# boguszjelinski/taxidispatcher

Hardware: AMD Instinct MI355X
Metric: NxN assignments/sec (higher is better)
Workload: dtype int32; 1 GPU; g1 N=16384: device cost write (4N^2 B) + exact assignment, total checked == optimum; n=16384, parallelism=single GPU

## Files before the change

taxidispatcher_amd/csrc/td_assign.hip:

```cpp
#include <dlfcn.h>
#include <limits.h>
#include <stdlib.h>

#include <type_traits>

#include "td_common.h"

using namespace td;

namespace {

template <typename CT>
struct Tr;
template <>
struct Tr<uint8_t> {
    using PT = int32_t;
    static constexpr int E = 16;
    static constexpr uint32_t SENT = 0xFFu;
    static constexpr int64_t LIMIT = 254;
    static constexpr int32_t BIG = 1 << 28;
    static constexpr int32_t KMAX = INT32_MAX;
};
template <>
struct Tr<uint16_t> {
// ... 830 lines not shown
        bk = s_k[wb];
        bp = s_p[wb];
        x = s_x[wb];
        for (int k = 0; k < 4; k++)
            if (k != wb && s_k[k] < x) x = s_k[k];
        if (bp != INT_MAX) {
            const int t1 = bp / E;
            int ch = t1 + rot;
            if (ch >= nchunks) ch -= nchunks;
            const int j1 = ch * E + (bp - t1 * E);
            const PT inc = (x == Tr<CT>::KMAX) ? (PT)0 : (PT)((x >> 1) - (bk >> 1));
            const bool owned = (bk & 1) != 0;
            if (j1 < n && (!(owned && inc == 0) || tie_evict)) {
                const PT newp = (P[j1] >> 1) + inc;
                atomicMax(&bid[j1], ((unsigned long long)newp << ROW_BITS) | (unsigned long long)(row + 1));
            }
        }
    }
    __syncthreads();
    }
}

template <typename PT>
__global__ __launch_bounds__(256) void k_assign(int n, int nrows, int row0, unsigned long long *__restrict__ bid,
                                                PT *__restrict__ pk, int *__restrict__ owner, int *__restrict__ r2c,
                                                int *__restrict__ ctl, int round, long long plimit = 0 )
{
    if (ctl[CTL_FLAG]) return;
    if (round > 0 && round < 60 && ctl[CTL_PROG + round - 1] == 0) return;
    const int j = blockIdx.x * blockDim.x + threadIdx.x;
    int cnt = 0;
    if (j < n) {
        const unsigned long long k = bid[j];
        if (k) {
            const int row = (int)(k & ((1ull << ROW_BITS) - 1)) - 1;
            const PT newp = (PT)(k >> ROW_BITS);
            if (plimit && (long long)(k >> ROW_BITS) >= plimit) atomicOr(&ctl[CTL_FLAG], 8);
            const int old = owner[j];
            const PT oldp = pk[j] >> 1;
            if (old >= row0 && old < row0 + nrows) r2c[old - row0] = -1;
            owner[j] = row;
            if (row >= row0 && row < row0 + nrows) r2c[row - row0] = j;
            pk[j] = (PT)(newp << 1) | (PT)1;
            bid[j] = 0ull;
            cnt = (old < 0 || newp > oldp) ? 1 : 0;
        }
    }
    const unsigned long long m = __ballot(cnt);
    if ((threadIdx.x & 63) == 0 && m) {
        if (round < 60) atomicAdd(&ctl[CTL_PROG + round], (int)__popcll(m));
    }
}

__device__ __forceinline__ int build_free_list(int n, const int *__restrict__ r2c, int *__restrict__ list, int want = -1)
{
    __shared__ int s_fl_w[16];
    __shared__ int s_fl_tot;
    const int T = blockDim.x, tid = threadIdx.x, lane = tid & 63, w = tid >> 6, nw = T >> 6;
    const int per = (n + T - 1) / T;
    const int lo = tid * per, hi = min(n, lo + per);
    int cnt = 0;
    const bool vec = (per & 3) == 0 && (reinterpret_cast<uintptr_t>(r2c) & 15) == 0;
    if (vec) {
        int r = lo;
#pragma unroll 4
        for (; r + 4 <= hi; r += 4) {
            const int4 x = *reinterpret_cast<const int4 *>(r2c + r);
            cnt += (x.x == want) + (x.y == want) + (x.z == want) + (x.w == want);
        }
        for (; r < hi; r++) cnt += (r2c[r] == want) ? 1 : 0;
    } else
        for (int r = lo; r < hi; r++) cnt += (r2c[r] == want) ? 1 : 0;
    int incl = cnt;
#pragma unroll
    for (int o = 1; o < 64; o <<= 1) {
        const int v = __shfl_up(incl, o);
        if (lane >= o) incl += v;
    }
    if (lane == 63) s_fl_w[w] = incl;
    __syncthreads();
    int base = 0;
    for (int k = 0; k < w; k++) base += s_fl_w[k];
    if (tid == T - 1) s_fl_tot = base + incl;
    int pos = base + incl - cnt;
    if (cnt) {
        if (vec) {
            int r = lo;
            for (; r + 4 <= hi; r += 4) {
                const int4 x = *reinterpret_cast<const int4 *>(r2c + r);
                if (x.x == want) list[pos++] = r;
                if (x.y == want) list[pos++] = r + 1;
                if (x.z == want) list[pos++] = r + 2;
                if (x.w == want) list[pos++] = r + 3;
            }
            for (; r < hi; r++)
                if (r2c[r] == want) list[pos++] = r;
        } else
            for (int r = lo; r < hi; r++)
                if (r2c[r] == want) list[pos++] = r;
    }
    __syncthreads();
    const int tot = s_fl_tot;
    __syncthreads();
    return tot;
}

__global__ __launch_bounds__(1024) void k_freelist(int n, const int *__restrict__ r2c, int *__restrict__ list,
                                                   int *__restrict__ ctl)
{
    if (ctl[CTL_FLAG]) return;
    const int cnt = build_free_list(n, r2c, list);
    if (threadIdx.x == 0) ctl[CTL_NFREE] = cnt;
}

#include "td_blocks.h"
#include "td_core_warm.h"

__device__ __forceinline__ void place_const_tail(int n, int *__restrict__ r2c, int *__restrict__ owner,
                                                 int *__restrict__ lista, int *__restrict__ listb,
                                                 int *__restrict__ ctl)
{
    if (ctl[CTL_NCONST] == 0) return;
    const int nr = build_free_list(n, r2c, lista, -2);
    if (nr == 0) return;
    const int nc = build_free_list(n, owner, listb, -1);
    if (nc != nr) {
        if (threadIdx.x == 0) atomicOr(&ctl[CTL_ERR], 8);
        return;
    }
    for (int k = threadIdx.x; k < nr; k += blockDim.x) {
        const int r = lista[k], j = listb[k];
        r2c[r] = j;
        owner[j] = r;
    }
}

__global__ __launch_bounds__(1024) void k_place_const(int n, int *__restrict__ r2c, int *__restrict__ owner,
                                                      int *__restrict__ lista, int *__restrict__ listb,
                                                      int *__restrict__ ctl, const int *__restrict__ gate_left = nullptr)
{
    if (ctl[CTL_FLAG]) return;
    if (gate_left && *gate_left != 0) return;
    place_const_tail(n, r2c, owner, lista, listb, ctl);
}

__device__ __forceinline__ void shape_decide(int n, int *__restrict__ ctl)
{
    int *sh = ctl + CTL_SHAPE;
    __threadfence();
    const int ncol = atomicAdd(&sh[0], 0);
    const int nrow = atomicAdd(&ctl[CTL_NCONST], 0);
    sh[1] = nrow;
    const int margin = n / 256 > 32 ? n / 256 : 32;
    if (ncol >= 16 && ncol - nrow >= margin) {
        sh[3] = 1;
        atomicOr(&ctl[CTL_FLAG], 4);
    }
}

__device__ __forceinline__ void shape_probe(int n, const int32_t *__restrict__ cost, int *__restrict__ ctl, int tickets)
{
    int *sh = ctl + CTL_SHAPE;
    const int t = blockIdx.x * blockDim.x + threadIdx.x;
    int cc = 0;
    long long rng = 0;
    if (t < n) {
        const int v0 = cost[t];
        int mn = v0, mx = v0;
#pragma unroll
        for (int k = 1; k < 16; k++) {
            const int v = cost[(int64_t)(((int64_t)k * n) >> 4) * n + t];
            mn = min(mn, v);
            mx = max(mx, v);
        }
        cc = (mn == mx) ? 1 : 0;
        rng = (long long)mx - (long long)mn;
    }
#pragma unroll
    for (int o = 32; o > 0; o >>= 1) {
        cc += __shfl_xor(cc, o);
        const long long orng = __shfl_xor(rng, o);
        rng = orng > rng ? orng : rng;
    }
    if ((threadIdx.x & 63) == 0) {
        if (cc) atomicAdd(&sh[0], cc);
        if (rng > 254) atomicMax(reinterpret_cast<unsigned long long *>(&sh[4]), (unsigned long long)rng);
    }
    __shared__ int s_last;
    __syncthreads();
    if (threadIdx.x == 0) {
        __threadfence();
        s_last = (atomicAdd(&sh[2], 1) == tickets - 1);
    }
    __syncthreads();
    if (s_last && threadIdx.x == 0) shape_decide(n, ctl);
// ... 1490 lines not shown
        for (int k = lane; k < rc->plen; k += 64) ok = ok && (touch[rc->path[k]] == r);
        for (int k = lane; k < rc->nS; k += 64) ok = ok && (pthm[rc->S_col[k]] >= r);
        if (__ballot(!ok)) continue;
        for (int k = lane; k < rc->nS; k += 64) {
            const int col = rc->S_col[k];
            const unsigned long long rv = atomicExch(&raise[col], 0ull);
            if (rv) {
                if (plimit && (long long)(pk[col] >> 1) + (long long)rv >= plimit) atomicOr(&ctl[CTL_FLAG], 8);
                pk[col] = pk[col] + (PT)((PT)rv << 1);
            }
        }
        if (lane == 0) pk[rc->endcol] = pk[rc->endcol] | (PT)1;
    }
    __syncthreads();
    const int nleft = build_free_list(n, r2c, list);
    if (tid == 0) s_nfree = nleft;
    __syncthreads();
    if (tid == 0) {
        ctl[CTL_NFREE] = s_nfree;
        if (!first && s_acc == 0) ctl[CTL_PSTOP] = 1;
        ctl[CTL_PACC] += s_acc;
    }
}

__device__ __forceinline__ void fin_record(const int *ctl, const unsigned long long *out, const int *left, unsigned int *ticket, int *rec)
{
    __shared__ int s_last;
    __syncthreads();
    if (threadIdx.x == 0) {
        __threadfence();
        s_last = atomicAdd(ticket, 1u) == gridDim.x - 1;
    }
    __syncthreads();
    if (!s_last) return;
    __threadfence();
    for (int k = threadIdx.x; k < CTL_ALL; k += blockDim.x) rec[k] = __hip_atomic_load(ctl + k, __ATOMIC_RELAXED, __HIP_MEMORY_SCOPE_AGENT);
    if (threadIdx.x == 0) {
        long long *rt = reinterpret_cast<long long *>(reinterpret_cast<char *>(rec) + FIN_OFF);
        rt[0] = (long long)__hip_atomic_load(out, __ATOMIC_RELAXED, __HIP_MEMORY_SCOPE_AGENT);
        rt[1] = (long long)__hip_atomic_load(out + 1, __ATOMIC_RELAXED, __HIP_MEMORY_SCOPE_AGENT);
        rec[REC_LEFT / sizeof(int)] = __hip_atomic_load(left, __ATOMIC_RELAXED, __HIP_MEMORY_SCOPE_AGENT);
        *ticket = 0u;
    }
}

template <bool GEN = false>
__global__ __launch_bounds__(256) void k_final(int n, int nrows, int row0, const int32_t *__restrict__ cost,
                                               const int *__restrict__ r2c, const int *__restrict__ owner,
                                               unsigned long long *__restrict__ out, int *__restrict__ ctl, int cost_is_transposed = 0,
                                               const CellSrc src = CellSrc(), const int *__restrict__ gate_left = nullptr,
                                               int *__restrict__ r2c_out = nullptr, unsigned int *__restrict__ ticket = nullptr,
                                               int *__restrict__ rec = nullptr)
{
    const bool go = !ctl[CTL_FLAG] && !(gate_left && *gate_left != 0);
    if (go) {
    long long s = 0;
    int bad = 0;
    for (int i = blockIdx.x * blockDim.x + threadIdx.x; i < nrows; i += gridDim.x * blockDim.x) {
        const int j = r2c[i];
        if (r2c_out) r2c_out[i] = j;
        if (j < 0 || j >= n || owner[j] != row0 + i)
            bad = 1;
        else
            s += GEN ? (long long)(cost_is_transposed ? src.cell(j, i) : src.cell(i, j))
                     : (long long)(cost_is_transposed ? cost[(int64_t)j * n + i] : cost[(int64_t)i * n + j]);
    }
#pragma unroll
    for (int o = 32; o > 0; o >>= 1) {
        s += __shfl_xor(s, o);
        bad |= __shfl_xor(bad, o);
    }
    if ((threadIdx.x & 63) == 0) {
        atomicAdd(&out[0], (unsigned long long)s);
        if (bad) atomicOr(&ctl[CTL_ERR], 4);
    }
    }
    if (rec) fin_record(ctl, out, gate_left, ticket, rec);
}

__global__ void k_pack_totals(const long long *__restrict__ tot2, const int *__restrict__ ctl, long long *__restrict__ out3)
{
    if (threadIdx.x == 0) {
        out3[0] = tot2[0];
        out3[1] = tot2[1];
        out3[2] = (long long)(ctl[CTL_ERR] != 0) + (long long)(ctl[CTL_FLAG] != 0);
    }
}

__global__ void k_r2c_from_owner(int n, int nrows, int row0, const int *__restrict__ owner, int *__restrict__ r2c)
{
    const int j = blockIdx.x * blockDim.x + threadIdx.x;
    if (j < n) {
        const int o = owner[j];
        if (o >= row0 && o < row0 + nrows) r2c[o - row0] = j;
    }
}

__global__ void k_const_mask(int row0, int nrows, const int *__restrict__ rconst, int *__restrict__ mask_full)
{
    const int i = blockIdx.x * blockDim.x + threadIdx.x;
    if (i < nrows && rconst[i]) mask_full[row0 + i] = 1;
}

__global__ __launch_bounds__(1024) void k_mark_const(int n, const int *__restrict__ mask, int *__restrict__ r2c_full, int *__restrict__ ctl)
{
    __shared__ int s_cnt;
    if (threadIdx.x == 0) s_cnt = 0;
    __syncthreads();
    int cnt = 0;
    for (int i = threadIdx.x; i < n; i += blockDim.x)
        if (mask[i]) {
            r2c_full[i] = -2;
            cnt++;
        }
#pragma unroll
    for (int o = 32; o > 0; o >>= 1) cnt += __shfl_xor(cnt, o);
    if ((threadIdx.x & 63) == 0 && cnt) atomicAdd(&s_cnt, cnt);
    __syncthreads();
    if (threadIdx.x == 0) ctl[CTL_NCONST] = s_cnt;
}

template <typename PT>
__global__ void k_price_io(int n, PT *pk, long long *plain, int set)
{
    const int j = blockIdx.x * blockDim.x + threadIdx.x;
    if (j < n) {
        if (set)
            pk[j] = (PT)((PT)plain[j] << 1) | (PT)1;
        else
            plain[j] = (long long)(pk[j] >> 1);
    }
}

__global__ void k_fill_i32(int *p, int count, int v)
{
    const int i = blockIdx.x * blockDim.x + threadIdx.x;
    if (i < count) p[i] = v;
}

template <typename CT>
__global__ __launch_bounds__(256) void k_dual(int n, int nrows, int row0, int nchunks, const CT *__restrict__ cc,
                                              const typename Tr<CT>::PT *__restrict__ pk,
                                              const int32_t *__restrict__ rowmin, unsigned long long *__restrict__ out,
                                              const int *__restrict__ gate_left = nullptr, const int *__restrict__ ctl = nullptr)
{
    using PT = typename Tr<CT>::PT;
    constexpr int E = Tr<CT>::E;
    if (gate_left && (*gate_left != 0 || ctl[CTL_FLAG] != 0)) return;
    const int lane = threadIdx.x & 63, w = threadIdx.x >> 6, nw = blockDim.x >> 6;
    const size_t pitch = (size_t)nchunks * E;
    long long acc = 0;
    for (int row = blockIdx.x * nw + w; row < nrows; row += gridDim.x * nw) {
        const CT *rp = cc + (size_t)row * pitch;
        PT m = Tr<CT>::KMAX;
        for (int ch = lane; ch < nchunks; ch += 64) {
            const uint4 cv = *reinterpret_cast<const uint4 *>(rp + (size_t)ch * E);
            uint32_t c[E];
            unpack<CT>(cv, c);
#pragma unroll
            for (int e = 0; e < E; e++) {
                const PT v = (PT)c[e] + (pk[(size_t)ch * E + e] >> 1);
                m = v < m ? v : m;
            }
        }
#pragma unroll
        for (int o = 32; o > 0; o >>= 1) {
            PT om = shfl_xor_t(m, o);
            m = om < m ? om : m;
        }
        if (lane == 0) acc += (long long)m + (long long)rowmin[row];
    }
    if (blockIdx.x == 0 && row0 == 0) {
        long long ps = 0;
        for (int j = threadIdx.x; j < n; j += blockDim.x) ps += (long long)(pk[j] >> 1);
#pragma unroll
        for (int o = 32; o > 0; o >>= 1) ps += __shfl_xor(ps, o);
        if (lane == 0) acc -= ps;
    }
    if (lane == 0 && acc != 0) atomicAdd(&out[1], (unsigned long long)acc);
}

}

struct td_shard {
    int n = 0, row0 = 0, nrows = 0;
    int bpc = 0;
    int64_t range = 0;
    int64_t fit_bound = -1;
    int nchunks = 0, npad = 0;
    const int32_t *d_cost = nullptr;
    Buf stage, cc, price, owner, r2c, r2c_full, bid, pred, list, rowmin, rconst, misc, psrec, tbuf, xbuf, fbuf;
    bool defer_const = false;
    int nconst = -1;
    const int32_t *probe = nullptr;
    bool placed = false;
    int64_t range_seen = -1;
    bool want_bid0 = false;
    bool bid0_done = false;
    Buf cmask;
    bool have_cmask = false;
    bool fused_t = false;
// ... 254 lines not shown
    HopCtl *hc = (HopCtl *)sv.hop.p;
    int *frl = (int *)sv.list.p, *fcl = (int *)sv.pred.p;
    const int *ctl = (const int *)sv.misc.p;
    if (gate && nb != 1) return fail(TD_EINTERNAL, "a gated two-hop pass takes one block");
    const int nseg = raw && window_zero ? (ncols_blk / 4 + 1023) / 1024 : 1;
    k_hop_lists<<<nb, 1024, 0, c.stream>>>(rpb, ncols_blk, col_lo, (const int *)sv.r2c.p, (const int *)sv.owner.p, frl, fcl, hc, ctl,
                                           gate ? g_hop_max_rows : 0, nseg > 1 ? (int *)sv.hoptab.p : nullptr);
    if (raw) {
        if (!sv.d_cost || sv.n % 4) return fail(TD_EINVAL, "two-hop pass on the int32 matrix: no matrix, or n %% 4 != 0");
        if (nseg > 1)
            k_hop_table<CT, true, true><<<nb * HOP_FMAX * nseg, 256, 0, c.stream>>>(
                sv.n, sv.nrows, sv.row0, sv.n / 4, rpb, ncols_blk, col_lo, g_hop_max_rows, 1, (const CT *)sv.d_cost, (const PT *)sv.price.p,
                (const int *)sv.owner.p, frl, fcl, hc, (int *)sv.hoptab.p, ctl, (const int32_t *)sv.rowmin.p, nseg);
        else
        k_hop_table<CT, true><<<nb * HOP_FMAX, 256, 0, c.stream>>>(sv.n, sv.nrows, sv.row0, sv.n / 4, rpb, ncols_blk, col_lo, g_hop_max_rows,
                                                                   window_zero ? 1 : 0, (const CT *)sv.d_cost, (const PT *)sv.price.p,
                                                                   (const int *)sv.owner.p, frl, fcl, hc, (int *)sv.hoptab.p, ctl,
                                                                   (const int32_t *)sv.rowmin.p);
    } else {
    k_hop_table<CT><<<nb * HOP_FMAX, 256, 0, c.stream>>>(sv.n, sv.nrows, sv.row0, sv.nchunks, rpb, ncols_blk, col_lo, g_hop_max_rows,
                                                         window_zero ? 1 : 0, (const CT *)sv.cc.p, (const PT *)sv.price.p,
                                                         (const int *)sv.owner.p, frl, fcl, hc, (int *)sv.hoptab.p, ctl);
    }
    const size_t match_lds = sizeof(uint32_t) * ((size_t)HOP_FMAX * HOP_FMAX + (size_t)((rpb + 31) / 32));
    if (match_lds > 150 * 1024) return fail(TD_EINVAL, "two-hop pass: a block of that many rows does not fit the LDS");
    TD_HIP(hipFuncSetAttribute((const void *)k_hop_match<PT>, hipFuncAttributeMaxDynamicSharedMemorySize, (int)match_lds));
    k_hop_match<PT><<<nb, HOP_MATCH_T, match_lds, c.stream>>>(
        sv.nrows, sv.row0, rpb, ncols_blk, col_lo, g_hop_max_rows, (PT *)sv.price.p, (int *)sv.owner.p, (int *)sv.r2c.p, ob, frl, fcl, hc,
        (const int *)sv.hoptab.p, (int *)sv.misc.p);
    TD_HIP(hipGetLastError());
    return TD_OK;
}

int sv_phase_a(Solver &sv, int hop_passes)
{
    Ctx &c = ctx();
    const int n = sv.n, nrows = sv.nrows;
    const int rpb = n / sv.zs_V, nb = nrows / rpb;
    const int col_lo = (sv.row0 / rpb) * rpb, col_hi = col_lo + nb * rpb;
    int rc;
    if ((rc = ensure(sv.ob, (size_t)sv.npad + 64))) return rc;
    if (!sv.ob_clear) TD_HIP(hipMemsetAsync(sv.ob.p, 0, (size_t)sv.npad, c.stream));
    sv.ob_clear = false;
    ProfScope ps(TD_K_BID);
    int *ctl = (int *)sv.misc.p;
    const int ga = (col_hi - col_lo + 255) / 256;
    unsigned long long *bid = (unsigned long long *)sv.bid.p;
    auto assign = [&]() {
        k_zs_assign<<<ga, 256, 0, c.stream>>>(col_lo, col_hi, nrows, sv.row0, bid, (int32_t *)sv.price.p, (int *)sv.owner.p, (int *)sv.r2c.p,
                                              (uint8_t *)sv.ob.p, ctl);
    };
    assign();
    for (int r = 1; r <= g_zs_rounds; r++) {
        k_zs_bid<<<std::min(nrows, c.n_cu * 16), 256, 0, c.stream>>>(nrows, sv.row0, sv.nchunks, rpb, (const uint8_t *)sv.cc.p,
                                                                     (const uint8_t *)sv.ob.p, (const int *)sv.r2c.p, bid, ctl, r, g_tie_evict);
        assign();
    }
    TD_HIP(hipGetLastError());
    for (int p = 0; p < hop_passes; p++)
        if ((rc = sv_hop_t<uint8_t>(sv, rpb, rpb, col_lo, nb, true, (uint8_t *)sv.ob.p))) return rc;
    if (getenv("TD_DEBUG") && hop_passes > 0) {
        HopCtl h;
        TD_HIP(hipMemcpyAsync(&h, sv.hop.p, sizeof(h), hipMemcpyDeviceToHost, c.stream));
        TD_HIP(hipStreamSynchronize(c.stream));
        fprintf(stderr, "[td] phase A: %d blocks of %d rows, %d local rounds; free rows / columns per block before the last two-hop pass:", nb, rpb, g_zs_rounds);
        for (int b = 0; b < nb; b++) fprintf(stderr, " %d/%d", h.nfr[b], h.nfc[b]);
        fprintf(stderr, " | matched %d, left %d\n", h.matched, h.left);
    }
    sv.zs_done = false;
    sv.bid0_done = false;
    sv.state_ready = true;
    return TD_OK;
}

template <typename CT>
int sv_begin_t(Solver &sv)
{
    Ctx &c = ctx();
    using PT = typename Tr<CT>::PT;
    const PT padkey = (PT)(Tr<CT>::BIG << 1) | (PT)1;
    k_init_state<PT><<<(std::max(sv.npad, (int)CTL_WORDS) + 255) / 256, 256, 0, c.stream>>>(
        sv.n, sv.npad, sv.nrows, (PT *)sv.price.p, padkey, (int *)sv.owner.p, (int *)sv.r2c.p,
        (unsigned long long *)sv.bid.p, (int *)sv.misc.p, sv.defer_const ? (const int *)sv.rconst.p : nullptr, sv.probe, 0, nullptr,
        g_one_trip ? (unsigned long long *)((char *)sv.misc.p + FIN_OFF) : nullptr);
    if (!g_one_trip) TD_HIP(hipMemsetAsync((char *)sv.misc.p + FIN_OFF, 0, 16, c.stream));
    TD_HIP(hipGetLastError());
    sv.began = true;
    return TD_OK;
}

template <typename CT>
int sv_bid_t(Solver &sv, int r, unsigned long long *keys)
{
    Ctx &c = ctx();
    using PT = typename Tr<CT>::PT;
    const int n = sv.n, nrows = sv.nrows;
    if (nrows == 0) return TD_OK;
    const size_t lds_prices = (size_t)sv.npad * sizeof(PT);
    const bool can_lds = lds_prices <= 128 * 1024 && n >= 2048 && nrows >= 1024;
    const int tie_evict = (r >= 1) ? g_tie_evict : 0;
    ProfScope ps(TD_K_BID);
    int *tied = (r == 0) ? (int *)sv.misc.p + CTL_TIED : nullptr;
    const bool sparse = sv.state_ready;
    if (can_lds && r < g_lds_rounds && !sparse) {
        if (lds_prices > 48 * 1024)
            (void)hipFuncSetAttribute((const void *)k_bid<CT, true>, hipFuncAttributeMaxDynamicSharedMemorySize, (int)lds_prices);
        const int grid = std::min((nrows + 15) / 16, c.n_cu * g_lds_grid);
// ... 1783 lines not shown
```

taxidispatcher_amd/csrc/td_blocks.h:

```cpp


struct HopCtl {
    int nfr[HOP_BMAX], nfc[HOP_BMAX];
    int left;
    int matched;
    int pad[2];
};

__device__ __forceinline__ uint32_t zs_zero_bytes(uint32_t w)
{
    return ~(((w & 0x7F7F7F7Fu) + 0x7F7F7F7Fu) | w | 0x7F7F7F7Fu);
}

__global__ __launch_bounds__(256) void k_zs_bid(int nrows, int row0, int nchunks, int rpb, const uint8_t *__restrict__ cc,
                                                const uint8_t *__restrict__ ob, const int *__restrict__ r2c,
                                                unsigned long long *__restrict__ bid, const int *__restrict__ ctl, int round,
                                                int tie_evict)
{
    __shared__ int s_best[4];
    if (ctl[CTL_FLAG]) return;
    const int tid = threadIdx.x, lane = tid & 63, w = tid >> 6;
    const int cpb = rpb >> 4;
    const size_t pitch = (size_t)nchunks * 16;
    for (int lrow = blockIdx.x; lrow < nrows; lrow += gridDim.x) {
        if (r2c[lrow] != -1) continue;
        const int row = row0 + lrow;
        const int c0 = (row / rpb) * cpb;
        const uint32_t hsh = ((uint32_t)row + 1u) * 0x9E3779B1u + (uint32_t)round * 0x85EBCA6Bu;
        const int rot = (int)(((uint64_t)(hsh ^ (hsh >> 15)) * (uint64_t)cpb) >> 32);
        const uint8_t *rp = cc + (size_t)lrow * pitch;
        int best = INT_MAX;
        for (int t = tid; t < cpb; t += 256) {
            int ch = t + rot;
            if (ch >= cpb) ch -= cpb;
            ch += c0;
            const uint4 cv = *reinterpret_cast<const uint4 *>(rp + (size_t)ch * 16);
            const uint4 ov = *reinterpret_cast<const uint4 *>(ob + (size_t)ch * 16);
            const uint32_t cw[4] = {cv.x, cv.y, cv.z, cv.w}, ow[4] = {ov.x, ov.y, ov.z, ov.w};
#pragma unroll
            for (int k = 0; k < 4; k++) {
                const uint32_t z = zs_zero_bytes(cw[k]);
                if (!z) continue;
                const uint32_t zf = z & zs_zero_bytes(ow[k]);
                const uint32_t pick = zf ? zf : z;
                const int cand = (zf ? 0 : (1 << 24)) | (t * 16 + k * 4 + (__builtin_ctz(pick) >> 3));
                best = min(best, cand);
            }
        }
#pragma unroll
        for (int o = 32; o > 0; o >>= 1) best = min(best, __shfl_xor(best, o));
        if (lane == 0) s_best[w] = best;
        __syncthreads();
        if (tid == 0) {
            best = min(min(s_best[0], s_best[1]), min(s_best[2], s_best[3]));
            if (best != INT_MAX) {
                const bool owned = (best >> 24) != 0;
                const int pos = best & 0xFFFFFF;
                int ch = (pos >> 4) + rot;
                if (ch >= cpb) ch -= cpb;
                const int j = (c0 + ch) * 16 + (pos & 15);
                if (!owned || tie_evict) atomicMax(&bid[j], (unsigned long long)(row + 1));
            }
        }
        __syncthreads();
    }
}

__global__ __launch_bounds__(256) void k_zs_assign(int col_lo, int col_hi, int nrows, int row0, unsigned long long *__restrict__ bid,
                                                   int32_t *__restrict__ pk, int *__restrict__ owner, int *__restrict__ r2c,
                                                   uint8_t *__restrict__ ob, const int *__restrict__ ctl)
{
    if (ctl[CTL_FLAG]) return;
    const int j = col_lo + blockIdx.x * blockDim.x + threadIdx.x;
    if (j >= col_hi) return;
    const unsigned long long k = bid[j];
    if (!k) return;
    const int row = (int)(k & ((1ull << ROW_BITS) - 1)) - 1;
    const int old = owner[j];
    if (old >= row0 && old < row0 + nrows) r2c[old - row0] = -1;
    owner[j] = row;
    if (row >= row0 && row < row0 + nrows) r2c[row - row0] = j;
    pk[j] = 1;
    ob[j] = 1;
    bid[j] = 0ull;
}

constexpr int HOP_NONE = INT_MAX;
__global__ __launch_bounds__(1024) void k_hop_lists(int rpb, int ncols_blk, int col_lo, const int *__restrict__ r2c,
                                                    const int *__restrict__ owner, int *__restrict__ frl, int *__restrict__ fcl,
                                                    HopCtl *__restrict__ hc, const int *__restrict__ ctl, int gate_max = 0,
                                                    int *__restrict__ tab_preset = nullptr)
{
    if (ctl[CTL_FLAG]) return;
    const int lb = blockIdx.x;
    if (gate_max > 0) {
        __shared__ int s_go;
        if (threadIdx.x == 0) {
            const int left = hc->left;
            s_go = left > 0 && left <= gate_max;
        }
        __syncthreads();
        if (!s_go) {
            if (threadIdx.x == 0) hc->nfr[lb] = 0, hc->nfc[lb] = 0;
            return;
        }
    }
    const int nfr = build_free_list(rpb, r2c + (size_t)lb * rpb, frl + (size_t)lb * rpb, -1);
    const int nfc = build_free_list(ncols_blk, owner + col_lo + (size_t)lb * ncols_blk, fcl + (size_t)lb * ncols_blk, -1);
    if (threadIdx.x == 0) {
        hc->nfr[lb] = nfr;
        hc->nfc[lb] = nfc;
        if (lb == 0) hc->left = 0, hc->matched = 0;
    }
    if (tab_preset) {
        int4 *t4 = reinterpret_cast<int4 *>(tab_preset + (size_t)lb * HOP_FMAX * HOP_FMAX);
        for (int k = threadIdx.x; k < min(nfr, HOP_FMAX) * (HOP_FMAX / 4); k += 1024) t4[k] = make_int4(HOP_NONE, HOP_NONE, HOP_NONE, HOP_NONE);
    }
}

template <typename CT, bool RAW = false, bool SPLIT = false>
__global__ __launch_bounds__(256) void k_hop_table(int n, int nrows, int row0, int nchunks, int rpb, int ncols_blk, int col_lo,
                                                   int max_rows, int window_zero, const CT *__restrict__ cc,
                                                   const typename Tr<CT>::PT *__restrict__ pk, const int *__restrict__ owner,
                                                   const int *__restrict__ frl, const int *__restrict__ fcl,
                                                   const HopCtl *__restrict__ hc, int *__restrict__ tab,
                                                   const int *__restrict__ ctl, const int32_t *__restrict__ rowmin = nullptr,
                                                   int nseg = 1)
{
    using PT = typename Tr<CT>::PT;
    constexpr int E = RAW ? 4 : Tr<CT>::E;
    __shared__ int s_tab[HOP_FMAX];
    constexpr int CHT = RAW ? 4 : 1;
    __shared__ int s_cand[256 * E * CHT];
    __shared__ int s_hr[256 * E * CHT], s_hj[256 * E * CHT];
    __shared__ int s_fc[HOP_FMAX];
    __shared__ int s_ncand, s_nhit;
    __shared__ long long s_v[4];
    constexpr int HU = 4;
    if (ctl[CTL_FLAG]) return;
    const int seg = SPLIT ? (int)blockIdx.x % nseg : 0, ba = SPLIT ? (int)blockIdx.x / nseg : (int)blockIdx.x;
    const int lb = ba / HOP_FMAX, a = ba % HOP_FMAX;
    const int nfr = hc->nfr[lb];
    if (nfr > max_rows || a >= min(nfr, HOP_FMAX)) return;
    const int tid = threadIdx.x, lane = tid & 63, w = tid >> 6;
    const int lrow = lb * rpb + frl[(size_t)lb * rpb + a];
    const size_t pitch = (size_t)nchunks * E;
    const unsigned char *rp = reinterpret_cast<const unsigned char *>(cc) + (size_t)lrow * pitch * (RAW ? 4 : sizeof(CT));
    const int32_t mn = RAW ? rowmin[lrow] : 0;
    auto cells = [&](const uint4 &raw, uint32_t *c) {
        if constexpr (RAW) {
            c[0] = (uint32_t)((int32_t)raw.x - mn), c[1] = (uint32_t)((int32_t)raw.y - mn);
            c[2] = (uint32_t)((int32_t)raw.z - mn), c[3] = (uint32_t)((int32_t)raw.w - mn);
        } else
            unpack<CT>(raw, c);
    };
    auto ecell = [&](int rl, int col) -> long long {
        if constexpr (RAW) return (long long)(uint32_t)(reinterpret_cast<const int32_t *>(cc)[(size_t)rl * pitch + col] - rowmin[rl]);
        else return (long long)(uint32_t)cc[(size_t)rl * pitch + col];
    };
    const int nfc = min(hc->nfc[lb], HOP_FMAX);
    const int cb = col_lo + lb * ncols_blk;
    if (tid < nfc) s_fc[tid] = fcl[(size_t)lb * ncols_blk + tid];
    int *tab_row = tab + ((size_t)lb * HOP_FMAX + a) * HOP_FMAX;
    if (!SPLIT && tid < HOP_FMAX) s_tab[tid] = INT_MAX;
    if (tid == 0) s_ncand = 0, s_nhit = 0;
    const int ch_lo = window_zero ? (col_lo + lb * ncols_blk) / E : 0;
    const int ch_n = window_zero ? (ncols_blk + E - 1) / E : nchunks;
    long long v = 0;
    if (!window_zero) {
        long long mv = LLONG_MAX;
        for (int t = tid; t < ch_n; t += 256) {
            uint32_t c[E];
            cells(*reinterpret_cast<const uint4 *>(rp + (size_t)(ch_lo + t) * 16), c);
            PT pv[E];
            const int j0 = (ch_lo + t) * E;
            if constexpr (sizeof(PT) == 4) {
                const int4 *pp = reinterpret_cast<const int4 *>(pk + j0);
#pragma unroll
                for (int q = 0; q < E / 4; q++) {
                    const int4 x = pp[q];
                    pv[4 * q + 0] = x.x, pv[4 * q + 1] = x.y, pv[4 * q + 2] = x.z, pv[4 * q + 3] = x.w;
                }
            } else {
#pragma unroll
                for (int e = 0; e < E; e++) pv[e] = pk[j0 + e];
            }
#pragma unroll
            for (int e = 0; e < E; e++)
                if (j0 + e < n) mv = min(mv, (long long)c[e] + (long long)(pv[e] >> 1));
        }
#pragma unroll
        for (int o = 32; o > 0; o >>= 1) {
            const long long ov = __shfl_xor(mv, o);
            mv = ov < mv ? ov : mv;
        }
        if (lane == 0) s_v[w] = mv;
        __syncthreads();
        v = min(min(s_v[0], s_v[1]), min(s_v[2], s_v[3]));
    }
    __syncthreads();
    for (int t0 = SPLIT ? seg * 256 * CHT : 0; t0 < (SPLIT ? min(ch_n, (seg + 1) * 256 * CHT) : ch_n); t0 += 256 * CHT) {
        uint4 raws[CHT];
#pragma unroll
        for (int u = 0; u < CHT; u++) {
            const int t = t0 + u * 256 + tid;
            if (t < ch_n) raws[u] = *reinterpret_cast<const uint4 *>(rp + (size_t)(ch_lo + t) * 16);
        }
#pragma unroll
        for (int u = 0; u < CHT; u++) {
        const int t = t0 + u * 256 + tid;
        if (t < ch_n) {
            const uint4 raw = raws[u];
            bool any = true;
            if constexpr (!RAW && sizeof(CT) == 1 && std::is_same<CT, uint8_t>::value)
                if (window_zero) any = (zs_zero_bytes(raw.x) | zs_zero_bytes(raw.y) | zs_zero_bytes(raw.z) | zs_zero_bytes(raw.w)) != 0;
// ... 22 lines not shown
        }
        }
        __syncthreads();
        const int nc = s_ncand;
        for (int k = tid; k < nc; k += 256) {
            const int j = s_cand[k], r = owner[j];
            if (r < row0 || r >= row0 + nrows) continue;
            if ((r - row0) / rpb != lb) continue;
            const int h = atomicAdd(&s_nhit, 1);
            s_hr[h] = r - row0, s_hj[h] = j;
        }
        __syncthreads();
        const int np = s_nhit * nfc;
        int *dst = SPLIT ? tab_row : s_tab;
        for (int p0 = 0; p0 < np; p0 += 256 * HU) {
            long long du[HU], dx[HU];
            int rg[HU], bb[HU];
            bool live[HU];
#pragma unroll
            for (int q = 0; q < HU; q++) {
                const int p = min(p0 + q * 256 + tid, np - 1);
                const int h = p / nfc, b = p - h * nfc;
                const int rl = s_hr[h], j = s_hj[h], jb = cb + s_fc[b];
                rg[q] = rl + row0, bb[q] = b;
                live[q] = SPLIT || s_tab[b] > rg[q];
                du[q] = dx[q] = 0;
                if (live[q]) {
                    du[q] = ecell(rl, j) + (long long)(pk[j] >> 1);
                    dx[q] = ecell(rl, jb) + (long long)(pk[jb] >> 1);
                }
            }
#pragma unroll
            for (int q = 0; q < HU; q++)
                if (live[q] && p0 + q * 256 + tid < np && du[q] == dx[q]) atomicMin(&dst[bb[q]], rg[q]);
        }
        __syncthreads();
        if (tid == 0) s_ncand = 0, s_nhit = 0;
        __syncthreads();
    }
    if (!SPLIT && tid < HOP_FMAX) tab_row[tid] = s_tab[tid] == INT_MAX ? -1 : s_tab[tid];
}

constexpr int HOP_MATCH_T = 256;
template <typename PT>
__global__ __launch_bounds__(HOP_MATCH_T) void k_hop_match(int nrows, int row0, int rpb, int ncols_blk, int col_lo, int max_rows,
                                                           PT *__restrict__ pk, int *__restrict__ owner, int *__restrict__ r2c,
                                                           uint8_t *__restrict__ ob, const int *__restrict__ frl,
                                                           const int *__restrict__ fcl, HopCtl *__restrict__ hc,
                                                           const int *__restrict__ tab, int *__restrict__ ctl)
{
    extern __shared__ uint32_t s_hop_dyn[];
    __shared__ int s_st[HOP_FMAX];
    __shared__ int s_win[HOP_FMAX][2];
    if (ctl[CTL_FLAG]) return;
    const int lb = blockIdx.x;
    const int nfr = hc->nfr[lb];
    const int tid = threadIdx.x;
    if (nfr == 0) return;
    if (nfr > max_rows) {
        if (tid == 0) atomicAdd(&hc->left, nfr);
        return;
    }
    const int na = min(nfr, HOP_FMAX), nc = min(hc->nfc[lb], HOP_FMAX);
    int *s_tab = reinterpret_cast<int *>(s_hop_dyn);
    uint32_t *s_usedr = s_hop_dyn + HOP_FMAX * HOP_FMAX;
    const int *fr = frl + (size_t)lb * rpb, *fc = fcl + (size_t)lb * ncols_blk;
    const int blk_row0 = row0 + lb * rpb;
    const int my_i = tid < na ? blk_row0 + fr[tid] : 0;
    {
        const int4 *src = reinterpret_cast<const int4 *>(tab + (size_t)lb * HOP_FMAX * HOP_FMAX);
        int4 *dst = reinterpret_cast<int4 *>(s_tab);
        auto norm = [&](int r, int col) { return (r == HOP_NONE || col >= nc) ? -1 : r; };
        for (int k = tid; k < na * (HOP_FMAX / 4); k += HOP_MATCH_T) {
            const int4 x = src[k];
            const int col = (k * 4) & (HOP_FMAX - 1);
            dst[k] = make_int4(norm(x.x, col), norm(x.y, col + 1), norm(x.z, col + 2), norm(x.w, col + 3));
        }
        for (int k = tid; k < (rpb + 31) / 32; k += HOP_MATCH_T) s_usedr[k] = 0u;
        if (tid < na) {
            const uint32_t hsh = ((uint32_t)my_i + 1u) * 0x9E3779B1u;
            s_st[tid] = nc ? (int)(((uint64_t)(hsh ^ (hsh >> 15)) * (uint64_t)nc) >> 32) : 0;
        }
    }
    __syncthreads();
    if (tid < 64) {
        const int lane = tid;
        auto entry = [&](int a, int col) -> int {
            const int r = s_tab[min(a, HOP_FMAX - 1) * HOP_FMAX + col];
            return a < na ? r : -1;
        };
        auto used = [&](int r) -> bool {
            const int rb = max(r - blk_row0, 0);
            const uint32_t word = s_usedr[rb >> 5];
            return r < 0 || ((word >> (rb & 31)) & 1u);
        };
        unsigned long long usedc0 = 0ull, usedc1 = 0ull;
        int done = 0, r_prev = -1;
        int ra0 = entry(0, lane), ra1 = entry(0, lane + 64);
        int rb0 = entry(1, lane), rb1 = entry(1, lane + 64);
        bool ua0 = used(ra0), ua1 = used(ra1);
        int st = s_st[0];
        for (int a = 0; a < na; a++) {
            const int rc0 = entry(a + 2, lane), rc1 = entry(a + 2, lane + 64);
            const bool ub0 = used(rb0), ub1 = used(rb1);
            const int st_nx = s_st[min(a + 1, HOP_FMAX - 1)];
            const unsigned long long m0 = __ballot(!ua0 && ra0 != r_prev) & ~usedc0;
            const unsigned long long m1 = __ballot(!ua1 && ra1 != r_prev) & ~usedc1;
            int rw = -1, cw = 0;
            if (m0 | m1) {
                const unsigned long long h0 = st < 64 ? m0 & (~0ull << st) : 0ull;
                const unsigned long long h1 = st < 64 ? m1 : m1 & (~0ull << (st - 64));
                if (h0 | h1) cw = h0 ? __builtin_ctzll(h0) : 64 + __builtin_ctzll(h1);
                else cw = m0 ? __builtin_ctzll(m0) : 64 + __builtin_ctzll(m1);
                rw = __builtin_amdgcn_readlane(cw < 64 ? ra0 : ra1, cw & 63);
                if (cw < 64) usedc0 |= 1ull << cw;
                else usedc1 |= 1ull << (cw - 64);
                r_prev = rw;
                done++;
            }
            if (lane == 0) {
                s_win[a][0] = rw, s_win[a][1] = cw;
                if (rw >= 0) {
                    const int rb = rw - blk_row0;
                    atomicOr(&s_usedr[rb >> 5], 1u << (rb & 31));
                }
            }
            __builtin_amdgcn_fence(__ATOMIC_ACQ_REL, "wavefront");
            ra0 = rb0, ra1 = rb1, ua0 = ub0, ua1 = ub1;
            rb0 = rc0, rb1 = rc1;
// ... 22 lines not shown
```

Baseline: 29.38 million assignments/s.

## Hoist control-flag loads and batch independent loads across small assignment kernels

Several small kernels (zero-slack bid, bid apply, hop free-list, hop table, hop match, final check, place_const) now issue their control-flag reads together with the first data loads, so the latencies overlap instead of running in series. k_zs_bid is remapped to one wavefront per row with no shared-memory barriers and two chunks in flight per lane. The grid grows to one block per four rows. The free-list builder fuses the row and column counting passes and their prefix scans into a single pass. This adds speculative loads, clamped indices and a larger launch grid, and it leans on empty asm statements to force load ordering.

```diff
diff --git a/taxidispatcher_amd/csrc/td_assign.hip b/taxidispatcher_amd/csrc/td_assign.hip
--- a/taxidispatcher_amd/csrc/td_assign.hip
+++ b/taxidispatcher_amd/csrc/td_assign.hip
@@ -906,16 +906,18 @@
     }
 }
 
-__device__ __forceinline__ int build_free_list(int n, const int *__restrict__ r2c, int *__restrict__ list, int want = -1)
-{
-    __shared__ int s_fl_w[16];
-    __shared__ int s_fl_tot;
-    const int T = blockDim.x, tid = threadIdx.x, lane = tid & 63, w = tid >> 6, nw = T >> 6;
+__device__ __forceinline__ bool free_list_vec(int n, const int *r2c)
+{
+    return (((n + (int)blockDim.x - 1) / (int)blockDim.x) & 3) == 0 && (reinterpret_cast<uintptr_t>(r2c) & 15) == 0;
+}
+
+__device__ __forceinline__ int free_list_count(int n, const int *__restrict__ r2c, int want)
+{
+    const int T = blockDim.x, tid = threadIdx.x;
     const int per = (n + T - 1) / T;
     const int lo = tid * per, hi = min(n, lo + per);
     int cnt = 0;
-    const bool vec = (per & 3) == 0 && (reinterpret_cast<uintptr_t>(r2c) & 15) == 0;
-    if (vec) {
+    if (free_list_vec(n, r2c)) {
         int r = lo;
 #pragma unroll 4
         for (; r + 4 <= hi; r += 4) {
@@ -925,6 +927,71 @@
         for (; r < hi; r++) cnt += (r2c[r] == want) ? 1 : 0;
     } else
         for (int r = lo; r < hi; r++) cnt += (r2c[r] == want) ? 1 : 0;
+    return cnt;
+}
+
+__device__ __forceinline__ void free_list_count2(int n, const int *__restrict__ a, int wanta, const int *__restrict__ b, int wantb,
+                                                 int &cnta, int &cntb)
+{
+    const int T = blockDim.x, tid = threadIdx.x;
+    const int per = (n + T - 1) / T;
+    const int lo = tid * per, hi = min(n, lo + per);
+    int ca = 0, cb = 0;
+    if ((n & 3) == 0 && free_list_vec(n, a) && free_list_vec(n, b)) {
+        for (int r = lo; r < hi; r += 16) {
+            int4 xa[4], xb[4];
+#pragma unroll
+            for (int q = 0; q < 4; q++) {
+                const int rr = min(r + 4 * q, hi - 4);
+                xa[q] = *reinterpret_cast<const int4 *>(a + rr), xb[q] = *reinterpret_cast<const int4 *>(b + rr);
+            }
+#pragma unroll
+            for (int q = 0; q < 4; q++)
+                if (r + 4 * q < hi) {
+                    ca += (xa[q].x == wanta) + (xa[q].y == wanta) + (xa[q].z == wanta) + (xa[q].w == wanta);
+                    cb += (xb[q].x == wantb) + (xb[q].y == wantb) + (xb[q].z == wantb) + (xb[q].w == wantb);
+                }
+        }
+    } else
+        for (int r = lo; r < hi; r += 4) {
+            int va[4], vb[4];
+#pragma unroll
+            for (int q = 0; q < 4; q++) va[q] = a[min(r + q, hi - 1)], vb[q] = b[min(r + q, hi - 1)];
+#pragma unroll
+            for (int q = 0; q < 4; q++)
+                if (r + q < hi) ca += va[q] == wanta, cb += vb[q] == wantb;
+        }
+    cnta = ca, cntb = cb;
+}
+
+__device__ __forceinline__ void free_list_fill(int n, const int *__restrict__ r2c, int *__restrict__ list, int want, int cnt, int pos)
+{
+    if (!cnt) return;
+    const int T = blockDim.x, tid = threadIdx.x;
+    const int per = (n + T - 1) / T;
+    const int lo = tid * per, hi = min(n, lo + per);
+    if (free_list_vec(n, r2c)) {
+        int r = lo;
+        for (; r + 4 <= hi; r += 4) {
+            const int4 x = *reinterpret_cast<const int4 *>(r2c + r);
+            if (x.x == want) list[pos++] = r;
+            if (x.y == want) list[pos++] = r + 1;
+            if (x.z == want) list[pos++] = r + 2;
+            if (x.w == want) list[pos++] = r + 3;
+        }
+        for (; r < hi; r++)
+            if (r2c[r] == want) list[pos++] = r;
+    } else
+        for (int r = lo; r < hi; r++)
+            if (r2c[r] == want) list[pos++] = r;
+}
+
+__device__ __forceinline__ int build_free_list(int n, const int *__restrict__ r2c, int *__restrict__ list, int want = -1)
+{
+    __shared__ int s_fl_w[16];
+    __shared__ int s_fl_tot;
+    const int T = blockDim.x, tid = threadIdx.x, lane = tid & 63, w = tid >> 6;
+    const int cnt = free_list_count(n, r2c, want);
     int incl = cnt;
 #pragma unroll
     for (int o = 1; o < 64; o <<= 1) {
@@ -936,27 +1003,35 @@
     int base = 0;
     for (int k = 0; k < w; k++) base += s_fl_w[k];
     if (tid == T - 1) s_fl_tot = base + incl;
-    int pos = base + incl - cnt;
-    if (cnt) {
-        if (vec) {
-            int r = lo;
-            for (; r + 4 <= hi; r += 4) {
-                const int4 x = *reinterpret_cast<const int4 *>(r2c + r);
-                if (x.x == want) list[pos++] = r;
-                if (x.y == want) list[pos++] = r + 1;
-                if (x.z == want) list[pos++] = r + 2;
-                if (x.w == want) list[pos++] = r + 3;
-            }
-            for (; r < hi; r++)
-                if (r2c[r] == want) list[pos++] = r;
-        } else
-            for (int r = lo; r < hi; r++)
-                if (r2c[r] == want) list[pos++] = r;
-    }
+    free_list_fill(n, r2c, list, want, cnt, base + incl - cnt);
     __syncthreads();
     const int tot = s_fl_tot;
     __syncthreads();
     return tot;
+}
+
+__device__ __forceinline__ void build_free_list2(int na, const int *__restrict__ a, int *__restrict__ lista, int wanta, int cnta,
+                                                 int nb, const int *__restrict__ b, int *__restrict__ listb, int wantb, int cntb,
+                                                 int &tota, int &totb)
+{
+    __shared__ int s_fl2_w[2][16];
+    __shared__ int s_fl2_tot[2];
+    const int T = blockDim.x, tid = threadIdx.x, lane = tid & 63, w = tid >> 6;
+    int ia = cnta, ib = cntb;
+#pragma unroll
+    for (int o = 1; o < 64; o <<= 1) {
+        const int va = __shfl_up(ia, o), vb = __shfl_up(ib, o);
+        if (lane >= o) ia += va, ib += vb;
+    }
+    if (lane == 63) s_fl2_w[0][w] = ia, s_fl2_w[1][w] = ib;
+    __syncthreads();
+    int basea = 0, baseb = 0;
+    for (int k = 0; k < w; k++) basea += s_fl2_w[0][k], baseb += s_fl2_w[1][k];
+    if (tid == T - 1) s_fl2_tot[0] = basea + ia, s_fl2_tot[1] = baseb + ib;
+    free_list_fill(na, a, lista, wanta, cnta, basea + ia - cnta);
+    free_list_fill(nb, b, listb, wantb, cntb, baseb + ib - cntb);
+    __syncthreads();
+    tota = s_fl2_tot[0], totb = s_fl2_tot[1];
 }
 
 __global__ __launch_bounds__(1024) void k_freelist(int n, const int *__restrict__ r2c, int *__restrict__ list,
@@ -993,8 +1068,11 @@
                                                       int *__restrict__ lista, int *__restrict__ listb,
                                                       int *__restrict__ ctl, const int *__restrict__ gate_left = nullptr)
 {
-    if (ctl[CTL_FLAG]) return;
-    if (gate_left && *gate_left != 0) return;
+    const int flag = __hip_atomic_load(&ctl[CTL_FLAG], __ATOMIC_RELAXED, __HIP_MEMORY_SCOPE_AGENT);
+    const int nconst = __hip_atomic_load(&ctl[CTL_NCONST], __ATOMIC_RELAXED, __HIP_MEMORY_SCOPE_AGENT);
+    const int left = gate_left ? *gate_left : 0;
+    asm volatile("" :: "v"(flag), "v"(nconst), "s"(left));
+    if (flag || left != 0 || nconst == 0) return;
     place_const_tail(n, r2c, owner, lista, listb, ctl);
 }
 
@@ -2591,18 +2669,26 @@
                                                int *__restrict__ r2c_out = nullptr, unsigned int *__restrict__ ticket = nullptr,
                                                int *__restrict__ rec = nullptr)
 {
-    const bool go = !ctl[CTL_FLAG] && !(gate_left && *gate_left != 0);
+    const int i0 = blockIdx.x * blockDim.x + threadIdx.x;
+    const int flag = __hip_atomic_load(&ctl[CTL_FLAG], __ATOMIC_RELAXED, __HIP_MEMORY_SCOPE_AGENT);
+    const int left = gate_left ? *gate_left : 0;
+    const int j0 = r2c[min(i0, nrows - 1)];
+    asm volatile("" :: "v"(flag), "s"(left), "v"(j0));
+    const bool go = !flag && left == 0;
     if (go) {
     long long s = 0;
     int bad = 0;
-    for (int i = blockIdx.x * blockDim.x + threadIdx.x; i < nrows; i += gridDim.x * blockDim.x) {
-        const int j = r2c[i];
+    for (int i = i0; i < nrows; i += gridDim.x * blockDim.x) {
+        const int j = i == i0 ? j0 : r2c[i];
         if (r2c_out) r2c_out[i] = j;
-        if (j < 0 || j >= n || owner[j] != row0 + i)
+        const int jc = min(max(j, 0), n - 1);
+        const int own = owner[jc];
+        long long cell = 0;
+        if constexpr (!GEN) cell = (long long)(cost_is_transposed ? cost[(int64_t)jc * n + i] : cost[(int64_t)i * n + jc]);
+        if (j < 0 || j >= n || own != row0 + i)
             bad = 1;
         else
-            s += GEN ? (long long)(cost_is_transposed ? src.cell(j, i) : src.cell(i, j))
-                     : (long long)(cost_is_transposed ? cost[(int64_t)j * n + i] : cost[(int64_t)i * n + j]);
+            s += GEN ? (long long)(cost_is_transposed ? src.cell(j, i) : src.cell(i, j)) : cell;
     }
 #pragma unroll
     for (int o = 32; o > 0; o >>= 1) {
@@ -2685,7 +2771,11 @@
 {
     using PT = typename Tr<CT>::PT;
     constexpr int E = Tr<CT>::E;
-    if (gate_left && (*gate_left != 0 || ctl[CTL_FLAG] != 0)) return;
+    if (gate_left) {
+        const int left = *gate_left, flag = ctl[CTL_FLAG];
+        asm volatile("" :: "s"(left), "s"(flag));
+        if (left != 0 || flag != 0) return;
+    }
     const int lane = threadIdx.x & 63, w = threadIdx.x >> 6, nw = blockDim.x >> 6;
     const size_t pitch = (size_t)nchunks * E;
     long long acc = 0;
@@ -3046,7 +3136,7 @@
     };
     assign();
     for (int r = 1; r <= g_zs_rounds; r++) {
-        k_zs_bid<<<std::min(nrows, c.n_cu * 16), 256, 0, c.stream>>>(nrows, sv.row0, sv.nchunks, rpb, (const uint8_t *)sv.cc.p,
+        k_zs_bid<<<(nrows + 3) / 4, 256, 0, c.stream>>>(nrows, sv.row0, sv.nchunks, rpb, (const uint8_t *)sv.cc.p,
                                                                      (const uint8_t *)sv.ob.p, (const int *)sv.r2c.p, bid, ctl, r, g_tie_evict);
         assign();
     }
diff --git a/taxidispatcher_amd/csrc/td_blocks.h b/taxidispatcher_amd/csrc/td_blocks.h
--- a/taxidispatcher_amd/csrc/td_blocks.h
+++ b/taxidispatcher_amd/csrc/td_blocks.h
@@ -12,57 +12,61 @@
     return ~(((w & 0x7F7F7F7Fu) + 0x7F7F7F7Fu) | w | 0x7F7F7F7Fu);
 }
 
+
 __global__ __launch_bounds__(256) void k_zs_bid(int nrows, int row0, int nchunks, int rpb, const uint8_t *__restrict__ cc,
                                                 const uint8_t *__restrict__ ob, const int *__restrict__ r2c,
                                                 unsigned long long *__restrict__ bid, const int *__restrict__ ctl, int round,
                                                 int tie_evict)
 {
-    __shared__ int s_best[4];
-    if (ctl[CTL_FLAG]) return;
-    const int tid = threadIdx.x, lane = tid & 63, w = tid >> 6;
+    const int lane = threadIdx.x & 63;
+    const int lrow = blockIdx.x * 4 + __builtin_amdgcn_readfirstlane(threadIdx.x >> 6);
+    const int flag = ctl[CTL_FLAG], col = r2c[min(lrow, nrows - 1)];
+    asm volatile("" :: "s"(flag), "s"(col));
+    if (flag || lrow >= nrows || col != -1) return;
     const int cpb = rpb >> 4;
     const size_t pitch = (size_t)nchunks * 16;
-    for (int lrow = blockIdx.x; lrow < nrows; lrow += gridDim.x) {
-        if (r2c[lrow] != -1) continue;
-        const int row = row0 + lrow;
-        const int c0 = (row / rpb) * cpb;
-        const uint32_t hsh = ((uint32_t)row + 1u) * 0x9E3779B1u + (uint32_t)round * 0x85EBCA6Bu;
-        const int rot = (int)(((uint64_t)(hsh ^ (hsh >> 15)) * (uint64_t)cpb) >> 32);
-        const uint8_t *rp = cc + (size_t)lrow * pitch;
-        int best = INT_MAX;
-        for (int t = tid; t < cpb; t += 256) {
-            int ch = t + rot;
+    const int row = row0 + lrow;
+    const int c0 = (row / rpb) * cpb;
+    const uint32_t hsh = ((uint32_t)row + 1u) * 0x9E3779B1u + (uint32_t)round * 0x85EBCA6Bu;
+    const int rot = (int)(((uint64_t)(hsh ^ (hsh >> 15)) * (uint64_t)cpb) >> 32);
+    const uint8_t *rp = cc + (size_t)lrow * pitch;
+    int best = INT_MAX;
+    for (int t0 = lane; t0 < cpb; t0 += 128) {
+        int t[2] = {t0, min(t0 + 64, cpb - 1)};
+        uint4 cv[2], ov[2];
+#pragma unroll
+        for (int u = 0; u < 2; u++) {
+            int ch = t[u] + rot;
             if (ch >= cpb) ch -= cpb;
             ch += c0;
-            const uint4 cv = *reinterpret_cast<const uint4 *>(rp + (size_t)ch * 16);
-            const uint4 ov = *reinterpret_cast<const uint4 *>(ob + (size_t)ch * 16);
-            const uint32_t cw[4] = {cv.x, cv.y, cv.z, cv.w}, ow[4] = {ov.x, ov.y, ov.z, ov.w};
-#pragma unroll
-            for (int k = 0; k < 4; k++) {
-                const uint32_t z = zs_zero_bytes(cw[k]);
+            cv[u] = *reinterpret_cast<const uint4 *>(rp + (size_t)ch * 16);
+            ov[u] = *reinterpret_cast<const uint4 *>(ob + (size_t)ch * 16);
+        }
+        asm volatile("" :: "v"(cv[0].x), "v"(cv[0].y), "v"(cv[0].z), "v"(cv[0].w), "v"(ov[0].x), "v"(ov[0].y), "v"(ov[0].z), "v"(ov[0].w),
+                     "v"(cv[1].x), "v"(cv[1].y), "v"(cv[1].z), "v"(cv[1].w), "v"(ov[1].x), "v"(ov[1].y), "v"(ov[1].z), "v"(ov[1].w));
+#pragma unroll
+        for (int u = 0; u < 2; u++) {
+            const uint32_t cw[4] = {cv[u].x, cv[u].y, cv[u].z, cv[u].w}, ow[4] = {ov[u].x, ov[u].y, ov[u].z, ov[u].w};
+#pragma unroll
+            for (int q = 0; q < 4; q++) {
+                const uint32_t z = zs_zero_bytes(cw[q]);
                 if (!z) continue;
-                const uint32_t zf = z & zs_zero_bytes(ow[k]);
+                const uint32_t zf = z & zs_zero_bytes(ow[q]);
                 const uint32_t pick = zf ? zf : z;
-                const int cand = (zf ? 0 : (1 << 24)) | (t * 16 + k * 4 + (__builtin_ctz(pick) >> 3));
+                const int cand = (zf ? 0 : (1 << 24)) | (t[u] * 16 + q * 4 + (__builtin_ctz(pick) >> 3));
                 best = min(best, cand);
             }
         }
-#pragma unroll
-        for (int o = 32; o > 0; o >>= 1) best = min(best, __shfl_xor(best, o));
-        if (lane == 0) s_best[w] = best;
-        __syncthreads();
-        if (tid == 0) {
-            best = min(min(s_best[0], s_best[1]), min(s_best[2], s_best[3]));
-            if (best != INT_MAX) {
-                const bool owned = (best >> 24) != 0;
-                const int pos = best & 0xFFFFFF;
-                int ch = (pos >> 4) + rot;
-                if (ch >= cpb) ch -= cpb;
-                const int j = (c0 + ch) * 16 + (pos & 15);
-                if (!owned || tie_evict) atomicMax(&bid[j], (unsigned long long)(row + 1));
-            }
-        }
-        __syncthreads();
+    }
+#pragma unroll
+    for (int o = 32; o > 0; o >>= 1) best = min(best, __shfl_xor(best, o));
+    if (lane == 0 && best != INT_MAX) {
+        const bool owned = (best >> 24) != 0;
+        const int pos = best & 0xFFFFFF;
+        int ch = (pos >> 4) + rot;
+        if (ch >= cpb) ch -= cpb;
+        const int j = (c0 + ch) * 16 + (pos & 15);
+        if (!owned || tie_evict) atomicMax(&bid[j], (unsigned long long)(row + 1));
     }
 }
 
@@ -70,13 +74,14 @@
                                                    int32_t *__restrict__ pk, int *__restrict__ owner, int *__restrict__ r2c,
                                                    uint8_t *__restrict__ ob, const int *__restrict__ ctl)
 {
-    if (ctl[CTL_FLAG]) return;
     const int j = col_lo + blockIdx.x * blockDim.x + threadIdx.x;
-    if (j >= col_hi) return;
-    const unsigned long long k = bid[j];
-    if (!k) return;
+    const int jc = min(j, col_hi - 1);
+    int flag = ctl[CTL_FLAG];
+    unsigned long long k = bid[jc];
+    int old = owner[jc];
+    asm volatile("" :: "s"(flag), "v"(k), "v"(old));
+    if (flag || j >= col_hi || !k) return;
     const int row = (int)(k & ((1ull << ROW_BITS) - 1)) - 1;
-    const int old = owner[j];
     if (old >= row0 && old < row0 + nrows) r2c[old - row0] = -1;
     owner[j] = row;
     if (row >= row0 && row < row0 + nrows) r2c[row - row0] = j;
@@ -91,22 +96,25 @@
                                                     HopCtl *__restrict__ hc, const int *__restrict__ ctl, int gate_max = 0,
                                                     int *__restrict__ tab_preset = nullptr)
 {
-    if (ctl[CTL_FLAG]) return;
     const int lb = blockIdx.x;
+    const int flag = __hip_atomic_load(&ctl[CTL_FLAG], __ATOMIC_RELAXED, __HIP_MEMORY_SCOPE_AGENT);
     if (gate_max > 0) {
-        __shared__ int s_go;
-        if (threadIdx.x == 0) {
-            const int left = hc->left;
-            s_go = left > 0 && left <= gate_max;
-        }
-        __syncthreads();
-        if (!s_go) {
+        const int left = __hip_atomic_load(&hc->left, __ATOMIC_RELAXED, __HIP_MEMORY_SCOPE_AGENT);
+        asm volatile("" :: "v"(flag), "v"(left));
+        if (flag) return;
+        if (!(left > 0 && left <= gate_max)) {
             if (threadIdx.x == 0) hc->nfr[lb] = 0, hc->nfc[lb] = 0;
             return;
         }
     }
-    const int nfr = build_free_list(rpb, r2c + (size_t)lb * rpb, frl + (size_t)lb * rpb, -1);
-    const int nfc = build_free_list(ncols_blk, owner + col_lo + (size_t)lb * ncols_blk, fcl + (size_t)lb * ncols_blk, -1);
+    const int *rs = r2c + (size_t)lb * rpb, *os = owner + col_lo + (size_t)lb * ncols_blk;
+    int cntr, cntc;
+    if (rpb == ncols_blk) free_list_count2(rpb, rs, -1, os, -1, cntr, cntc);
+    else cntr = free_list_count(rpb, rs, -1), cntc = free_list_count(ncols_blk, os, -1);
+    asm volatile("" :: "v"(cntr), "v"(cntc));
+    if (flag) return;
+    int nfr, nfc;
+    build_free_list2(rpb, rs, frl + (size_t)lb * rpb, -1, cntr, ncols_blk, os, fcl + (size_t)lb * ncols_blk, -1, cntc, nfr, nfc);
     if (threadIdx.x == 0) {
         hc->nfr[lb] = nfr;
         hc->nfc[lb] = nfc;
@@ -137,13 +145,17 @@
     __shared__ int s_ncand, s_nhit;
     __shared__ long long s_v[4];
     constexpr int HU = 4;
-    if (ctl[CTL_FLAG]) return;
     const int seg = SPLIT ? (int)blockIdx.x % nseg : 0, ba = SPLIT ? (int)blockIdx.x / nseg : (int)blockIdx.x;
     const int lb = ba / HOP_FMAX, a = ba % HOP_FMAX;
-    const int nfr = hc->nfr[lb];
+    const int tid = threadIdx.x, lane = tid & 63, w = tid >> 6;
+    int flag = ctl[CTL_FLAG];
+    int nfr = hc->nfr[lb], nfc_all = hc->nfc[lb];
+    int fr_a = frl[(size_t)lb * rpb + min(a, rpb - 1)];
+    int fc_t = fcl[(size_t)lb * ncols_blk + min(tid & (HOP_FMAX - 1), ncols_blk - 1)];
+    asm volatile("" :: "s"(flag), "s"(nfr), "s"(nfc_all), "s"(fr_a), "v"(fc_t));
+    if (flag) return;
     if (nfr > max_rows || a >= min(nfr, HOP_FMAX)) return;
-    const int tid = threadIdx.x, lane = tid & 63, w = tid >> 6;
-    const int lrow = lb * rpb + frl[(size_t)lb * rpb + a];
+    const int lrow = lb * rpb + fr_a;
     const size_t pitch = (size_t)nchunks * E;
     const unsigned char *rp = reinterpret_cast<const unsigned char *>(cc) + (size_t)lrow * pitch * (RAW ? 4 : sizeof(CT));
     const int32_t mn = RAW ? rowmin[lrow] : 0;
@@ -158,9 +170,9 @@
         if constexpr (RAW) return (long long)(uint32_t)(reinterpret_cast<const int32_t *>(cc)[(size_t)rl * pitch + col] - rowmin[rl]);
         else return (long long)(uint32_t)cc[(size_t)rl * pitch + col];
     };
-    const int nfc = min(hc->nfc[lb], HOP_FMAX);
+    const int nfc = min(nfc_all, HOP_FMAX);
     const int cb = col_lo + lb * ncols_blk;
-    if (tid < nfc) s_fc[tid] = fcl[(size_t)lb * ncols_blk + tid];
+    if (tid < nfc) s_fc[tid] = fc_t;
     int *tab_row = tab + ((size_t)lb * HOP_FMAX + a) * HOP_FMAX;
     if (!SPLIT && tid < HOP_FMAX) s_tab[tid] = INT_MAX;
     if (tid == 0) s_ncand = 0, s_nhit = 0;
@@ -289,29 +301,50 @@
     extern __shared__ uint32_t s_hop_dyn[];
     __shared__ int s_st[HOP_FMAX];
     __shared__ int s_win[HOP_FMAX][2];
-    if (ctl[CTL_FLAG]) return;
+    constexpr int HOP_TAB_U = 4;
     const int lb = blockIdx.x;
-    const int nfr = hc->nfr[lb];
     const int tid = threadIdx.x;
+    const int *fr = frl + (size_t)lb * rpb, *fc = fcl + (size_t)lb * ncols_blk;
+    const int4 *src = reinterpret_cast<const int4 *>(tab + (size_t)lb * HOP_FMAX * HOP_FMAX);
+    int flag = ctl[CTL_FLAG];
+    int nfr = hc->nfr[lb], nfc_all = hc->nfc[lb];
+    int fr_t = fr[min(tid & (HOP_FMAX - 1), rpb - 1)];
+    int4 x0[HOP_TAB_U];
+#pragma unroll
+    for (int q = 0; q < HOP_TAB_U; q++) x0[q] = src[tid + q * HOP_MATCH_T];
+    asm volatile("" :: "s"(flag), "s"(nfr), "s"(nfc_all), "v"(fr_t), "v"(x0[0].x), "v"(x0[0].y), "v"(x0[0].z), "v"(x0[0].w),
+                 "v"(x0[1].x), "v"(x0[1].y), "v"(x0[1].z), "v"(x0[1].w), "v"(x0[2].x), "v"(x0[2].y), "v"(x0[2].z), "v"(x0[2].w),
+                 "v"(x0[3].x), "v"(x0[3].y), "v"(x0[3].z), "v"(x0[3].w));
+    static_assert(HOP_TAB_U == 4, "the operand list above");
+    if (flag) return;
     if (nfr == 0) return;
     if (nfr > max_rows) {
         if (tid == 0) atomicAdd(&hc->left, nfr);
         return;
     }
-    const int na = min(nfr, HOP_FMAX), nc = min(hc->nfc[lb], HOP_FMAX);
+    const int na = min(nfr, HOP_FMAX), nc = min(nfc_all, HOP_FMAX);
     int *s_tab = reinterpret_cast<int *>(s_hop_dyn);
     uint32_t *s_usedr = s_hop_dyn + HOP_FMAX * HOP_FMAX;
-    const int *fr = frl + (size_t)lb * rpb, *fc = fcl + (size_t)lb * ncols_blk;
     const int blk_row0 = row0 + lb * rpb;
-    const int my_i = tid < na ? blk_row0 + fr[tid] : 0;
+    const int my_i = tid < na ? blk_row0 + fr_t : 0;
     {
-        const int4 *src = reinterpret_cast<const int4 *>(tab + (size_t)lb * HOP_FMAX * HOP_FMAX);
         int4 *dst = reinterpret_cast<int4 *>(s_tab);
         auto norm = [&](int r, int col) { return (r == HOP_NONE || col >= nc) ? -1 : r; };
-        for (int k = tid; k < na * (HOP_FMAX / 4); k += HOP_MATCH_T) {
-            const int4 x = src[k];
+        auto stage = [&](int k, const int4 &x) {
             const int col = (k * 4) & (HOP_FMAX - 1);
             dst[k] = make_int4(norm(x.x, col), norm(x.y, col + 1), norm(x.z, col + 2), norm(x.w, col + 3));
+        };
+        const int nq = na * (HOP_FMAX / 4);
+#pragma unroll
+        for (int q = 0; q < HOP_TAB_U; q++)
+            if (tid + q * HOP_MATCH_T < nq) stage(tid + q * HOP_MATCH_T, x0[q]);
+        for (int k0 = tid + HOP_TAB_U * HOP_MATCH_T; k0 < nq; k0 += HOP_TAB_U * HOP_MATCH_T) {
+            int4 x[HOP_TAB_U];
+#pragma unroll
+            for (int q = 0; q < HOP_TAB_U; q++) x[q] = src[min(k0 + q * HOP_MATCH_T, nq - 1)];
+#pragma unroll
+            for (int q = 0; q < HOP_TAB_U; q++)
+                if (k0 + q * HOP_MATCH_T < nq) stage(k0 + q * HOP_MATCH_T, x[q]);
         }
         for (int k = tid; k < (rpb + 31) / 32; k += HOP_MATCH_T) s_usedr[k] = 0u;
         if (tid < na) {
```

After: 30.62 million assignments/s (median of 6 runs). 4.2% higher.
